# aszepieniec/stark-anatomy

Hardware: AMD Instinct MI355X
Metric: ntt_field_elements_per_sec (higher is better)
Workload: dtype u128; 1 GPU; ntt_fwd_inv_2^20_1gpu; log2n=20, parallelism=single, passes_per_transform=2

## Files before the change

### stark-anatomy_amd/csrc/core.h

```cpp
#pragma once
#include <hip/hip_runtime.h>
#include <dlfcn.h>
#include <cstdio>
#include <cstdlib>
#include <cstring>
#include <algorithm>
#include <atomic>
#include <chrono>
#include <cerrno>
#include <thread>
#include <sys/random.h>
#include <deque>
#include <functional>
#include <future>
#include <map>
#include <mutex>
#include <string>
#include <tuple>
#include <vector>

#pragma GCC visibility push(default)
#include "../../include/starkcore.h"
#pragma GCC visibility pop
#include "ntt_plan.h"

namespace sc { struct FoldIn; }
using namespace sc;

struct sc_vec {
    Fe* d;
    uint64_t n;
    bool owned = true;
};
struct sc_later {
    int slot;
    uint64_t seq;
    hipStream_t st;
};
struct sc_merkle {
    uint64_t* d_levels;
    uint64_t N;
    int logN;
    int slot = -1;
    uint64_t seq = 0;
    hipStream_t st = nullptr;
    bool have_root = false;
    bool lazy = false;
    uint8_t root[64] = {};
};

struct sc_merkle_forest {
    uint64_t* d_levels;
    uint64_t N, count;
    int logN;
    uint64_t* h_roots = nullptr;
    Fe* d_cm = nullptr;
    hipEvent_t done = nullptr;
    hipStream_t st = nullptr;
    bool have_roots = false;
};

namespace sci {

struct DevBuf {
    void* p = nullptr;
    size_t bytes = 0;
};

struct PlanKey {
    int logn;
    uint64_t lo, hi;
    bool operator<(const PlanKey& o) const { return std::tie(logn, lo, hi) < std::tie(o.logn, o.lo, o.hi); }
};
struct PlanTables {
    Fe* mt = nullptr;
    int mt_log = 0;
    Fe* tl = nullptr;
    Fe* th = nullptr;
    Fe* th_ninv = nullptr;
    struct Direct { int logA, logR; bool scaled; Fe* d; };
    std::vector<Direct> direct;
    uint64_t last_use = 0;
};
struct OuterKey {
    uint64_t lo, hi, order, len, batch, col_base;
    int ninv;
    bool operator<(const OuterKey& o) const { return std::tie(lo, hi, order, len, batch, col_base, ninv) < std::tie(o.lo, o.hi, o.order, o.len, o.batch, o.col_base, o.ninv); }
};
struct OuterTable {
    Fe* d = nullptr;
    uint64_t last_use = 0;
};
struct PowKey {
    uint64_t lo, hi, hi_count;
    bool operator<(const PowKey& o) const { return std::tie(lo, hi, hi_count) < std::tie(o.lo, o.hi, o.hi_count); }
};
struct PowTables {
    Fe* lo = nullptr;
    Fe* hi = nullptr;
    uint64_t last_use = 0;
};

struct Ctx {
    bool init = false;
    int device = -1;
    hipStream_t stream = nullptr;
    std::string err;
    NttTuning tuning;
    std::map<PlanKey, PlanTables> plans;
    std::map<PowKey, PowTables> pows;
    std::map<OuterKey, OuterTable> outers;
    uint64_t tick = 0;
    bool foreign_streams = false;
    int small_divisor_direct = 1;
    int div_cols_launch_log = 26;
    int tree_cols_launch_log = 26;
    int eval_chunk_log = 8;
    int eval_points_across_min = 32;
    int eval_across_min_products_log = 26;
    int rescue_tree_split_max_nodes = -1;
    int div_cols_chunk = 0;
    std::vector<hipStream_t> seen_streams;
    DevBuf scratch[8];
    std::map<hipStream_t, DevBuf> ntt_work;
    std::map<hipStream_t, DevBuf> ntt_flags;
    int fast_fixups = 1;
    int num_cus = 256;
    int xcd_remap = 1;
    int fixed_shapes = 1;
    int prio_balance = -1;
    int wave_local = 1;
    unsigned long long* trace = nullptr;
    int forest_four_lane_wgs = 256;
    int merkle_big_nlev = 2;
    int fri_tail = -1;
    int fri_tail_stall = -1;
    size_t verify_stage_bytes = 64ull << 20;
    uint8_t* root_slots = nullptr;
    uint8_t* later_words = nullptr;
    uint64_t root_seq = 0;
    std::vector<int> free_root_slots;
};
constexpr int ROOT_SLOTS = 256;
constexpr size_t ROOT_SLOT_BYTES = 128;
constexpr size_t LATER_WORD_BYTES = 128;
constexpr long SPIN_POLLS = 40000000;

struct PendingFree {
    void* p;
    size_t bytes;
    std::vector<hipEvent_t> evs;
};
#define HIPCHK(expr)                                                                                          \
    do {                                                                                                      \
        hipError_t _e = (expr);                                                                               \
        if (_e != hipSuccess) return fail(SC_ERR_HIP, std::string(#expr) + ": " + hipGetErrorString(_e));     \
    } while (0)

#define SCCHK(expr)              \
    do {                         \
        int _rc = (expr);        \
        if (_rc != SC_OK) return _rc; \
    } while (0)

struct NttOpts {
    uint64_t in_limit = ~0ull;
    const PowTables* coset = nullptr;
    uint32_t cols = 1;
    uint64_t col_stride_in = 0;
};
constexpr uint64_t COLS_ELEMS_PER_LAUNCH = 1ull << 26;
constexpr uint64_t SMALL_DIVISOR = 8;

constexpr uint64_t FUSE_MAX_W = 1ull << 17;

enum BuildMode { BUILD_SYNC = 0, BUILD_ASYNC = 1, BUILD_NOROOT = 2 };

extern Ctx g;
extern std::mutex g_mu;
extern hipStream_t g_comm_stream_for_free;
extern std::future<void> g_rand_worker;
extern size_t g_rand_prefetched;
extern std::multimap<size_t, void*> g_pool;
extern size_t g_pool_bytes, g_pool_cap;
extern std::deque<PendingFree> g_pending;
extern std::vector<hipEvent_t> g_event_pool;

void reap_pending(bool block);
hipError_t pool_alloc(void** p, size_t bytes);
void pool_free(void* p, size_t bytes);
void pool_clear();
hipEvent_t event_get();
int fail(int code, const std::string& msg);
int ensure_init();
int grow_buffer(DevBuf& b, size_t bytes, void** out);
inline int scratch(int slot, size_t bytes, void** out) { return grow_buffer(g.scratch[slot], bytes, out); }
int check_root(Fe root, uint64_t n);
int build_pow_table(Fe** out, uint64_t count, Fe base_m, uint64_t step, Fe scale_m, hipStream_t st);
void free_plans();
int evict_outer_tables();
int get_plan(Fe root, int logn, bool need_ninv, hipStream_t st, PlanTables** out);
inline NttTables tables_of(const PlanTables& t) {
    NttTables tb;
    tb.mt = t.mt; tb.mt_log = t.mt_log; tb.tl = t.tl; tb.th = t.th;
    return tb;
}
int get_pow(Fe base, uint64_t count, hipStream_t st, PowTables** out);
int plan_batched_direct(NttPlanDesc& d, BatchKind kind, int loglen, int logbatch, PlanTables* pt, const Fe* in, Fe* work, Fe* out, BatchExtras ex, hipStream_t st, bool* ok);
int run_plan(NttPlanDesc& d, hipStream_t st);
int ntt_device(const Fe* d_in, Fe* d_out, int logn, Fe root, bool inverse_scale, const NttOpts& o, hipStream_t st);
Fe root_inverse(Fe root, uint64_t n);
int ntt_any(const Fe* d_in, Fe* d_out, uint64_t n, Fe root, bool inverse, const NttOpts& o, hipStream_t st);
int upload(void* d, const void* h, size_t bytes, hipStream_t st);
int download(void* h, const void* d, size_t bytes, hipStream_t st);
int pointwise_div_device(const Fe* a, const Fe* b, Fe* out, uint64_t n, hipStream_t st);
int pointwise_div_enqueue(const Fe* a, const Fe* b, Fe* out, uint64_t n, hipStream_t st, uint32_t* flag);
int gather_device(const Fe* v, const uint64_t* d_idx, uint64_t k, Fe* d_out, hipStream_t st);
int read_small_polled(const void* d_src, size_t bytes, hipStream_t st, void* host_out);
bool upload_small(void* d_dst, const void* host, size_t bytes, hipStream_t st);

int merkle_climb(uint64_t* levels, uint64_t N, int lvl, hipStream_t st, volatile uint64_t* host = nullptr, uint64_t seq = 0, bool* published = nullptr);
int merkle_finish(uint64_t* levels, uint64_t width, hipStream_t st);
int root_slot_get();
int merkle_build_device(const Fe* d_elems, uint64_t N, uint8_t root_out[64], sc_merkle** tree, hipStream_t st, BuildMode mode = BUILD_SYNC, const FoldIn* fold = nullptr);
int merkle_root_wait(sc_merkle* t, bool from_free = false);
void root_poll_unlocked(std::unique_lock<std::mutex>& lk, const sc_merkle* t);
int fold_prepare(const Fe* d_in, uint64_t N, Fe alpha, Fe offset, Fe omega, Fe* d_out, hipStream_t st, FoldIn* f);
int fold_device(const Fe* d_in, uint64_t N, Fe alpha, Fe offset, Fe omega, Fe* d_out, hipStream_t st);
int fold_and_build(const Fe* d_in, uint64_t N, Fe alpha, Fe offset, Fe omega, Fe* d_out, sc_merkle** tree, hipStream_t st);
int fold_constants(uint64_t N, Fe offset, Fe omega, hipStream_t st, PowTables** pw_out, Fe* i2o_m_out);
int host_pool_get(size_t bytes, void** out);
int host_pool_put(void* p);
bool host_pool_holds(const void* p, size_t bytes);
int verify_stage_buffer(size_t bytes, uint8_t** out);

Fe canonical_root(int logn);
Fe ninv_scaled(int logn, int j);
int ntt_cols(const Fe* in, Fe* out, int loglen, int logbatch, bool inverse, hipStream_t st);

constexpr size_t SEEN_STREAMS = 8;
inline hipStream_t pick_stream(void* s) {
    if (s && (hipStream_t)s != g.stream) {
        g.foreign_streams = true;
        hipStream_t st = (hipStream_t)s;
        if (g.seen_streams.size() <= SEEN_STREAMS && std::find(g.seen_streams.begin(), g.seen_streams.end(), st) == g.seen_streams.end())
            g.seen_streams.push_back(st);
    }
    return s ? (hipStream_t)s : g.stream;
}
inline void release_after_streams(void* p, size_t bytes) {
    if (!p) return;
    if (g.seen_streams.size() > SEEN_STREAMS) {
        (void)hipDeviceSynchronize();
        g.seen_streams.clear();
        pool_free(p, bytes);
        return;
    }
    PendingFree f{p, bytes, {}};
    auto mark = [&](hipStream_t st) -> bool {
        if (hipStreamQuery(st) == hipSuccess) return true;
        (void)hipGetLastError();
        hipEvent_t e = event_get();
        if (!e) { (void)hipStreamSynchronize(st); (void)hipGetLastError(); return true; }
        if (hipEventRecord(e, st) != hipSuccess) { (void)hipGetLastError(); g_event_pool.push_back(e); return false; }
        f.evs.push_back(e);
        return true;
    };
    if (g.stream) (void)mark(g.stream);
    if (g_comm_stream_for_free) (void)mark(g_comm_stream_for_free);
    for (size_t i = 0; i < g.seen_streams.size();) {
        if (mark(g.seen_streams[i])) ++i;
        else g.seen_streams.erase(g.seen_streams.begin() + i);
    }
    if (f.evs.empty()) { pool_free(p, bytes); return; }
    g_pending.push_back(std::move(f));
    reap_pending(false);
}
inline Fe fe_from(const uint64_t v[2]) { return Fe{v[0], v[1]}; }
inline bool is_pow2(uint64_t n) { return n && !(n & (n - 1)); }
// ... 29 lines not shown
```

### stark-anatomy_amd/csrc/core.hip

```cpp
#include "core.h"


template <int LOGE> struct PassThreads { static constexpr int value = LOGE >= 4 ? 256 : (LOGE == 3 ? 512 : 1024); };

template <int LOGE>
__global__ void __launch_bounds__(PassThreads<LOGE>::value) ntt_pass_kernel(const PassParams P, uint32_t ntiles, int xcd_remap) {
    extern __shared__ __attribute__((aligned(16))) unsigned char smem_raw[];
    Fe* lds = reinterpret_cast<Fe*>(smem_raw);
    uint32_t wg = blockIdx.x, colbits = 0;
    if (P.col_enable) { colbits = (wg >> P.col_tiles_log) << P.col_tiles_log; wg -= colbits; }
    uint32_t tile = wg;
    if (xcd_remap) tile = (wg & 7u) * (ntiles >> 3) + (wg >> 3);
    tile |= colbits;
    Fe* tw = lds + (1u << (P.logR + P.logC));
    tile_twiddles_to_lds(P, P.logR, threadIdx.x, blockDim.x, tw);
    __syncthreads();
    const int nrounds = (P.logR + LOGE - 1) / LOGE;
    int sh = P.logR;
    for (int r = 0; r < nrounds; ++r) {
        const int s = (r == 0) ? (P.logR - LOGE * (nrounds - 1)) : LOGE;
        sh -= s;
        ntt_round_dispatch<LOGE>(P, s, sh, r == 0, tile, threadIdx.x, lds, tw);
        if (r + 1 < nrounds) __syncthreads();
    }
}

constexpr int TRACE_STAMPS = 16;
template <int LOGE, int GLR, int GLC, bool TRACE, bool ALT = false>
__global__ void __launch_bounds__(1 << (GLR + GLC - LOGE)) ntt_pass_kernel_fixed(const PassParams P, uint32_t ntiles, int xcd_remap, int wave_local) {
    extern __shared__ __attribute__((aligned(16))) unsigned char smem_raw[];
    Fe* lds = reinterpret_cast<Fe*>(smem_raw);
    unsigned long long* trow = nullptr;
    if constexpr (TRACE) {
        if (P.trace) {
            trow = P.trace + ((size_t)blockIdx.x * (blockDim.x >> 6) + (threadIdx.x >> 6)) * TRACE_STAMPS;
            if ((threadIdx.x & 63u) == 0) { trow[0] = __builtin_amdgcn_s_memtime(); trow[15] = __builtin_amdgcn_s_memrealtime(); }
        }
    }
    uint32_t wg = blockIdx.x, colbits = 0;
    if (P.col_enable) { colbits = (wg >> P.col_tiles_log) << P.col_tiles_log; wg -= colbits; }
    uint32_t tile = wg;
    if (xcd_remap) tile = (wg & 7u) * (ntiles >> 3) + (wg >> 3);
    tile |= colbits;
    Fe* tw = lds + (1u << (GLR + GLC));
    auto stamp = [&](int i) {
        if constexpr (TRACE) {
            if (trow) {
                if (i == 2) __builtin_amdgcn_s_waitcnt(0);
                if ((threadIdx.x & 63u) == 0 && i < 13) trow[i] = __builtin_amdgcn_s_memtime();
            }
        }
    };
    auto sync = [] { __syncthreads(); };
    auto wsync = [] { __builtin_amdgcn_fence(__ATOMIC_RELEASE, "wavefront"); __builtin_amdgcn_wave_barrier(); __builtin_amdgcn_fence(__ATOMIC_ACQUIRE, "wavefront"); };
    FixedRounds<LOGE, GLR, GLC, 0, ALT>::run(P, tile, threadIdx.x, lds, tw, sync, wsync, stamp, wave_local != 0);
    if constexpr (TRACE) {
        if (trow && (threadIdx.x & 63u) == 0) { __builtin_amdgcn_s_waitcnt(0); trow[14] = __builtin_amdgcn_s_memtime(); trow[13] = __builtin_amdgcn_s_memrealtime(); }
    }
}

template <int GLR, int GLC>
__device__ __forceinline__ uint32_t fixed8_tile(const PassParams& P, uint32_t index, uint32_t ntiles, int xcd_remap) {
    uint32_t wg = index, colbits = 0;
    if (P.col_enable) { colbits = (wg >> P.col_tiles_log) << P.col_tiles_log; wg -= colbits; }
    uint32_t tile = wg;
    if (xcd_remap) tile = (wg & 7u) * (ntiles >> 3) + (wg >> 3);
    return tile | colbits;
}
template <int GLR, int GLC>
__global__ void __launch_bounds__(1 << (GLR + GLC - 3)) __attribute__((amdgpu_waves_per_eu(4)))
ntt_pass_kernel_fixed8(const PassParams P, uint32_t ntiles, int xcd_remap, int wave_local, uint32_t* flags) {
    extern __shared__ __attribute__((aligned(16))) unsigned char smem_raw[];
    Fe* lds = reinterpret_cast<Fe*>(smem_raw);
    const uint32_t tile = fixed8_tile<GLR, GLC>(P, blockIdx.x, ntiles, xcd_remap);
    Fe* tw = lds + (1u << (GLR + GLC));
    auto stamp = [](int) {};
    auto sync = [] { __syncthreads(); };
    auto wsync = [] { __builtin_amdgcn_fence(__ATOMIC_RELEASE, "wavefront"); __builtin_amdgcn_wave_barrier(); __builtin_amdgcn_fence(__ATOMIC_ACQUIRE, "wavefront"); };
    rare_t rare = 0;
    FixedRounds<3, GLR, GLC, 0, false, true>::run(P, tile, threadIdx.x, lds, tw, sync, wsync, stamp, wave_local != 0, rare);
    if (rare_any(rare)) Round<3, 3, GLR, GLC>::store_word_at(flags + blockIdx.x, 0u, 1u);
}

template <int GLR, int GLC>
__global__ void __launch_bounds__(1 << (GLR + GLC - 3)) __attribute__((amdgpu_waves_per_eu(4)))
ntt_pass_redo8_kernel(const PassParams P, uint32_t ntiles, int xcd_remap, int wave_local, uint32_t* flags, int all) {
    extern __shared__ __attribute__((aligned(16))) unsigned char smem_raw[];
    if (!all && flags[blockIdx.x] == 0) return;
    Fe* lds = reinterpret_cast<Fe*>(smem_raw);
    Fe* tw = lds + (1u << (GLR + GLC));
    auto stamp = [](int) {};
    auto sync = [] { __syncthreads(); };
    auto wsync = [] { __builtin_amdgcn_fence(__ATOMIC_RELEASE, "wavefront"); __builtin_amdgcn_wave_barrier(); __builtin_amdgcn_fence(__ATOMIC_ACQUIRE, "wavefront"); };
    FixedRounds<3, GLR, GLC, 0, false>::run(P, fixed8_tile<GLR, GLC>(P, blockIdx.x, ntiles, xcd_remap), threadIdx.x, lds, tw, sync, wsync, stamp, wave_local != 0);
    if (!all) __syncthreads();
    if (threadIdx.x == 0) flags[blockIdx.x] = 0;
}

__global__ void __launch_bounds__(256) pow_table_kernel(Fe* out, uint64_t count, Fe base_m, uint64_t step, Fe scale_m) {
    uint64_t i = (uint64_t)blockIdx.x * blockDim.x + threadIdx.x;
    if (i < count) out[i] = pow_table_entry(base_m, i, step, scale_m);
}

__global__ void __launch_bounds__(256) twiddle_table_kernel(Fe* out, int logB, uint64_t count, uint64_t scale_exp, const Fe* __restrict__ tl, const Fe* __restrict__ th) {
    uint64_t i = (uint64_t)blockIdx.x * blockDim.x + threadIdx.x;
    if (i >= count) return;
    uint64_t k = i >> logB, b = i & ((1ull << logB) - 1);
    out[i] = pow2level(tl, th, b * k * scale_exp);
}

__global__ void __launch_bounds__(256) pointwise_mul_kernel(const Fe* __restrict__ a, const Fe* __restrict__ b, Fe* __restrict__ out, uint64_t n) {
    uint64_t i = (uint64_t)blockIdx.x * blockDim.x + threadIdx.x;
    if (i < n) out[i] = fe_mul(a[i], b[i]);
}

template <int K>
__global__ void __launch_bounds__(256) pointwise_div_kernel(const Fe* __restrict__ a, const Fe* __restrict__ b, Fe* __restrict__ out, uint64_t n, uint32_t* flag) {
    const uint64_t nthreads = (uint64_t)gridDim.x * blockDim.x;
    const uint64_t t = (uint64_t)blockIdx.x * blockDim.x + threadIdx.x;
    Fe bm[K], pre[K];
    Fe acc = fe_mont_one();
    bool zero = false;
#pragma unroll
    for (int k = 0; k < K; ++k) {
        uint64_t i = t + (uint64_t)k * nthreads;
        Fe v = (i < n) ? b[i] : fe_one();
        zero |= fe_is_zero(v);
        bm[k] = to_mont(v);
        pre[k] = acc;
        acc = mont_mul(acc, bm[k]);
    }
    if (zero) atomicOr(flag, 1u);
    Fe inv = mont_inv(acc);
#pragma unroll
    for (int k = K - 1; k >= 0; --k) {
        uint64_t i = t + (uint64_t)k * nthreads;
        Fe ik = mont_mul(inv, pre[k]);
        inv = mont_mul(inv, bm[k]);
        if (i < n) out[i] = mont_mul(a[i], ik);
    }
}

__global__ void __launch_bounds__(256) short_poly_coset_kernel(const Fe* __restrict__ b, uint32_t nb, Fe off_m, const Fe* __restrict__ tl, const Fe* __restrict__ th, Fe* __restrict__ out, uint64_t order) {
    const uint64_t i = (uint64_t)blockIdx.x * blockDim.x + threadIdx.x;
    if (i >= order) return;
    const Fe x_m = mont_mul(off_m, pow2level(tl, th, i));
    Fe acc = b[nb - 1];
    for (uint32_t k = nb - 1; k-- > 0;) acc = fe_add(mont_mul(acc, x_m), b[k]);
    out[i] = acc;
}

__global__ void __launch_bounds__(256) scale_pow_kernel(const Fe* __restrict__ in, Fe* __restrict__ out, uint64_t n, const Fe* __restrict__ lo, const Fe* __restrict__ hi) {
    uint64_t i = (uint64_t)blockIdx.x * blockDim.x + threadIdx.x;
    if (i < n) out[i] = mont_mul(in[i], pow2level(lo, hi, i));
}

__global__ void __launch_bounds__(256) scale_slab_kernel(const Fe* __restrict__ in, Fe* __restrict__ out, uint64_t rows, int logcols, uint64_t row_len, uint64_t col_base,
                                                         const Fe* __restrict__ lo, const Fe* __restrict__ hi) {
    uint64_t t = (uint64_t)blockIdx.x * blockDim.x + threadIdx.x;
    if (t >= (rows << logcols)) return;
    uint64_t r = t >> logcols, c = t & ((1ull << logcols) - 1);
    out[t] = mont_mul(in[t], pow2level(lo, hi, r * row_len + col_base + c));
}

__global__ void __launch_bounds__(256) axpy_shift_kernel(Fe* __restrict__ acc, const Fe* __restrict__ src, uint64_t n_src, uint64_t shift, Fe w_m) {
    uint64_t j = (uint64_t)blockIdx.x * blockDim.x + threadIdx.x;
    if (j >= n_src) return;
    acc[shift + j] = fe_add(acc[shift + j], mont_mul(src[j], w_m));
}

constexpr int DEGREE_PER_THREAD = 4;
constexpr unsigned DEGREE_MAX_BLOCKS = 2048;
constexpr int DEGREE_SLOTS = 8;
__global__ void __launch_bounds__(256) vec_degree_kernel(const Fe* __restrict__ v, uint64_t n, long long* out) {
    const uint64_t step = (uint64_t)gridDim.x * (256 * DEGREE_PER_THREAD);
    long long best = -1;
    for (uint64_t base = (uint64_t)blockIdx.x * (256 * DEGREE_PER_THREAD) + threadIdx.x; base - threadIdx.x < n; base += step) {
        Fe x[DEGREE_PER_THREAD];
#pragma unroll
        for (int k = 0; k < DEGREE_PER_THREAD; ++k) {
            const uint64_t i = base + 256u * k;
            x[k] = i < n ? v[i] : Fe{0, 0};
        }
#pragma unroll
        for (int k = 0; k < DEGREE_PER_THREAD; ++k) {
            const unsigned long long lanes = __ballot(!fe_is_zero(x[k]));
            if (lanes) best = (long long)(base - (threadIdx.x & 63u) + 256u * k + (63 - __clzll((long long)lanes)));
        }
    }
    __shared__ long long wave_best[4];
    if ((threadIdx.x & 63u) == 0) wave_best[threadIdx.x >> 6] = best;
    __syncthreads();
    if (threadIdx.x == 0) {
        long long m = wave_best[0];
#pragma unroll
        for (int w = 1; w < 4; ++w) m = wave_best[w] > m ? wave_best[w] : m;
        if (m >= 0) atomicMax(out + (blockIdx.x & (DEGREE_SLOTS - 1)), m);
    }
}
__global__ void __launch_bounds__(256) vec_degree_cols_kernel(const Fe* __restrict__ v, uint64_t n, uint64_t ld, uint32_t per_col, long long* out) {
    const uint64_t col = blockIdx.x / per_col;
    const uint32_t part = blockIdx.x - (uint32_t)col * per_col;
    const Fe* __restrict__ w = v + col * ld;
    const uint64_t step = (uint64_t)per_col * (256 * DEGREE_PER_THREAD);
    long long best = -1;
    for (uint64_t base = (uint64_t)part * (256 * DEGREE_PER_THREAD) + threadIdx.x; base - threadIdx.x < n; base += step) {
        Fe x[DEGREE_PER_THREAD];
#pragma unroll
        for (int k = 0; k < DEGREE_PER_THREAD; ++k) {
            const uint64_t i = base + 256u * k;
            x[k] = i < n ? w[i] : Fe{0, 0};
        }
#pragma unroll
        for (int k = 0; k < DEGREE_PER_THREAD; ++k) {
            const unsigned long long lanes = __ballot(!fe_is_zero(x[k]));
            if (lanes) best = (long long)(base - (threadIdx.x & 63u) + 256u * k + (63 - __clzll((long long)lanes)));
        }
    }
    __shared__ long long wave_best[4];
    if ((threadIdx.x & 63u) == 0) wave_best[threadIdx.x >> 6] = best;
    __syncthreads();
    if (threadIdx.x == 0) {
        long long m = wave_best[0];
#pragma unroll
        for (int k = 1; k < 4; ++k) m = wave_best[k] > m ? wave_best[k] : m;
        if (m >= 0) atomicMax(out + col, m);
    }
}
static int degree_read(void* fl, hipStream_t st, long long* deg) {
    long long slots[DEGREE_SLOTS];
    SCCHK(read_small_polled(fl, sizeof slots, st, slots));
    long long m = -1;
    for (int i = 0; i < DEGREE_SLOTS; ++i) m = slots[i] > m ? slots[i] : m;
    *deg = m;
    return SC_OK;
}
static inline unsigned degree_blocks(uint64_t n) {
    const uint64_t b = (n + 256 * DEGREE_PER_THREAD - 1) / (256 * DEGREE_PER_THREAD);
    return (unsigned)(b < DEGREE_MAX_BLOCKS ? (b ? b : 1) : DEGREE_MAX_BLOCKS);
}

__global__ void __launch_bounds__(256) mpoly_eval_kernel(const Fe* __restrict__ vals_m, uint32_t nvars, uint64_t n, const uint8_t* __restrict__ exps,
                                                        const Fe* __restrict__ coef_m, uint32_t nterms, Fe* __restrict__ out, const uint64_t* __restrict__ where) {
    uint64_t i = (uint64_t)blockIdx.x * blockDim.x + threadIdx.x;
    if (i >= n) return;
    Fe acc{0, 0};
    for (uint32_t t = 0; t < nterms; ++t) {
        Fe p = coef_m[t];
        const uint8_t* e = exps + (size_t)t * nvars;
// ... 227 lines not shown
    HIPCHK(hipMalloc((void**)out, count * sizeof(Fe)));
    unsigned blocks = (unsigned)((count + 255) / 256);
    hipLaunchKernelGGL(pow_table_kernel, dim3(blocks), dim3(256), 0, st, *out, count, base_m, step, scale_m);
    HIPCHK(hipGetLastError());
    return SC_OK;
}

void free_plan_tables(PlanTables& t) {
    hipFree(t.mt); hipFree(t.tl); hipFree(t.th);
    if (t.th_ninv) hipFree(t.th_ninv);
    for (const PlanTables::Direct& e : t.direct) hipFree(e.d);
}

void free_plans() {
    for (auto& kv : g.plans) free_plan_tables(kv.second);
    g.plans.clear();
    for (auto& kv : g.pows) { hipFree(kv.second.lo); hipFree(kv.second.hi); }
    g.pows.clear();
    for (auto& kv : g.outers) hipFree(kv.second.d);
    g.outers.clear();
}

constexpr uint64_t PIN_WINDOW = 64;
constexpr size_t PLAN_CAP = 256, POW_CAP = 64;

template <class Map, class FreeFn>
int evict_tables(Map& m, size_t cap, FreeFn free_entry) {
    if (m.size() < cap) return SC_OK;
    std::vector<std::pair<uint64_t, typename Map::iterator>> old;
    for (auto it = m.begin(); it != m.end(); ++it)
        if (it->second.last_use + PIN_WINDOW < g.tick) old.emplace_back(it->second.last_use, it);
    if (old.empty()) return SC_OK;
    std::sort(old.begin(), old.end(), [](const auto& a, const auto& b) { return a.first < b.first; });
    size_t drop = cap / 4 ? cap / 4 : 1;
    if (drop > old.size()) drop = old.size();
    HIPCHK(hipDeviceSynchronize());
    for (size_t i = 0; i < drop; ++i) { free_entry(old[i].second->second); m.erase(old[i].second); }
    return SC_OK;
}

int get_plan(Fe root, int logn, bool need_ninv, hipStream_t st, PlanTables** out) {
    PlanKey key{logn, root.lo, root.hi};
    auto it = g.plans.find(key);
    bool built = false;
    ++g.tick;
    if (it == g.plans.end()) {
        SCCHK(evict_tables(g.plans, PLAN_CAP, free_plan_tables));
        const uint64_t n = 1ull << logn;
        Fe rm = to_mont(root);
        const TableSizes sz = table_sizes(logn);
        PlanTables t;
        t.mt_log = sz.mt_log;
        SCCHK(build_pow_table(&t.mt, sz.mt, rm, n >> sz.mt_log, fe_mont_one(), st));
        SCCHK(build_pow_table(&t.tl, sz.tl, rm, 1, fe_mont_one(), st));
        SCCHK(build_pow_table(&t.th, sz.th, rm, 4096, fe_mont_one(), st));
        it = g.plans.emplace(key, t).first;
        built = true;
    }
    if (need_ninv && !it->second.th_ninv) {
        const uint64_t n = 1ull << logn;
        Fe ninv_m = mont_inv(to_mont(Fe{n, 0}));
        SCCHK(build_pow_table(&it->second.th_ninv, table_sizes(logn).th, to_mont(root), 4096, ninv_m, st));
        built = true;
    }
    if (built) HIPCHK(hipStreamSynchronize(st));
    it->second.last_use = g.tick;
    *out = &it->second;
    return SC_OK;
}

int get_pow(Fe base, uint64_t count, hipStream_t st, PowTables** out) {
    uint64_t hi_count = (count >> 12) + 1;
    uint64_t hc = 1; while (hc < hi_count) hc <<= 1;
    PowKey key{base.lo, base.hi, hc};
    auto it = g.pows.find(key);
    ++g.tick;
    if (it == g.pows.end()) {
        SCCHK(evict_tables(g.pows, POW_CAP, [](PowTables& t) { hipFree(t.lo); hipFree(t.hi); }));
        Fe bm = to_mont(base);
        PowTables t;
        SCCHK(build_pow_table(&t.lo, 4096, bm, 1, fe_mont_one(), st));
        SCCHK(build_pow_table(&t.hi, hc, bm, 4096, fe_mont_one(), st));
        HIPCHK(hipStreamSynchronize(st));
        it = g.pows.emplace(key, t).first;
    }
    it->second.last_use = g.tick;
    *out = &it->second;
    return SC_OK;
}

int direct_twiddles(PlanTables* pt, const NttPlanDesc& d, int i, bool scaled, hipStream_t st, const Fe** out) {
    const DirectTable t = direct_table(d, i, scaled);
    *out = nullptr;
    if (t.logR + t.logB > g.tuning.direct_tw_max_log) return SC_OK;
    for (const PlanTables::Direct& e : pt->direct)
        if (e.logA == t.logA && e.logR == t.logR && e.scaled == t.scaled) { *out = e.d; return SC_OK; }
    const uint64_t count = 1ull << (t.logR + t.logB);
    Fe* p;
    HIPCHK(hipMalloc((void**)&p, count * sizeof(Fe)));
    pt->direct.push_back({t.logA, t.logR, t.scaled, p});
    hipLaunchKernelGGL(twiddle_table_kernel, dim3((unsigned)((count + 255) / 256)), dim3(256), 0, st, p, t.logB, count, 1ull << t.logA,
                       pt->tl, t.scaled ? pt->th_ninv : pt->th);
    HIPCHK(hipGetLastError());
    HIPCHK(hipStreamSynchronize(st));
    *out = p;
    return SC_OK;
}

int plan_batched_direct(NttPlanDesc& d, BatchKind kind, int loglen, int logbatch, PlanTables* pt, const Fe* in, Fe* work, Fe* out, BatchExtras ex, hipStream_t st, bool* ok) {
    const NttTables tb = tables_of(*pt);
    *ok = plan_batched(d, kind, loglen, logbatch, tb, in, work, out, g.tuning, ex);
    if (!*ok || d.npasses != 2) return SC_OK;
    SCCHK(direct_twiddles(pt, d, 0, false, st, &ex.inner_twd));
    if (ex.inner_twd) *ok = plan_batched(d, kind, loglen, logbatch, tb, in, work, out, g.tuning, ex);
    return SC_OK;
}

int pass_flags(hipStream_t st, uint32_t nwg, uint32_t** out) {
    DevBuf& b = g.ntt_flags[st];
    const void* before = b.p;
    const size_t had = b.bytes;
    void* p;
    SCCHK(grow_buffer(b, (size_t)nwg * sizeof(uint32_t), &p));
    if (p != before || b.bytes != had) HIPCHK(hipMemsetAsync(p, 0, b.bytes, st));
    *out = (uint32_t*)p;
    return SC_OK;
}

template <int LOGE>
int launch_pass(const NttPassDesc& pd, hipStream_t st) {
    int remap = (g.xcd_remap && pd.ntiles >= 16 && (pd.ntiles & 7u) == 0) ? 1 : 0;
    const PassKernel k = pass_kernel(pd, g.fixed_shapes != 0);
    if constexpr (LOGE == 2) {
        if (k.kind == PK_FIXED4) {
            const int lr = pd.p.logR, lc = pd.p.logC;
#define SC_LAUNCH_FIXED(LR, LC, TR, ALT) \
    hipLaunchKernelGGL((ntt_pass_kernel_fixed<2, LR, LC, TR, ALT>), dim3(pd.ntiles * pd.cols), dim3(pd.threads), pd.lds_bytes, st, pd.p, pd.ntiles, remap, g.wave_local)
#define SC_FIXED(LR, LC)                                                          \
            if (lr == LR && lc == LC) {                                           \
                if (k.trace) SC_LAUNCH_FIXED(LR, LC, true, false);                \
                else if (k.alt) SC_LAUNCH_FIXED(LR, LC, false, true);             \
                else SC_LAUNCH_FIXED(LR, LC, false, false);                       \
                return SC_OK;                                                     \
            }
            SC_FIXED4_SHAPES(SC_FIXED)
#undef SC_FIXED
        }
    }
    if constexpr (LOGE == 3) {
        if (k.kind == PK_FIXED8) {
            const int lr = pd.p.logR, lc = pd.p.logC;
            const uint32_t nwg = pd.ntiles * pd.cols;
            const bool fast = g.fast_fixups != 0 && fast_pass_ok(pd.p) && !pass_in_place(pd);
            const int all = (!fast || g.fast_fixups == 2) ? 1 : 0;
            uint32_t* flags;
            SCCHK(pass_flags(st, nwg, &flags));
#define SC_FIXED8(LR, LC)                                                                                                                                   \
            if (lr == LR && lc == LC) {                                                                                                                     \
                if (fast) hipLaunchKernelGGL((ntt_pass_kernel_fixed8<LR, LC>), dim3(nwg), dim3(pd.threads), pd.lds_bytes, st, pd.p, pd.ntiles, remap, g.wave_local, flags); \
                hipLaunchKernelGGL((ntt_pass_redo8_kernel<LR, LC>), dim3(nwg), dim3(pd.threads), pd.lds_bytes, st, pd.p, pd.ntiles, remap, g.wave_local, flags, all); \
                return SC_OK;                                                                                                                               \
            }
            SC_FIXED8_SHAPES(SC_FIXED8)
#undef SC_FIXED8
        }
    }
    hipLaunchKernelGGL(ntt_pass_kernel<LOGE>, dim3(pd.ntiles * pd.cols), dim3(pd.threads), pd.lds_bytes, st, pd.p, pd.ntiles, remap);
    return SC_OK;
}

int run_plan(NttPlanDesc& d, hipStream_t st) {
    size_t trace_off = 0;
    for (int i = 0; i < d.npasses; ++i) {
        d.pass[i].p.prio_balance = pass_prio_balance(d.pass[i], g.prio_balance, g.num_cus);
        d.pass[i].p.trace = g.trace ? g.trace + trace_off : nullptr;
        trace_off += (size_t)d.pass[i].ntiles * d.pass[i].cols * (d.pass[i].threads >> 6) * TRACE_STAMPS;
        switch (d.pass[i].loge) {
            case 1: SCCHK(launch_pass<1>(d.pass[i], st)); break;
            case 2: SCCHK(launch_pass<2>(d.pass[i], st)); break;
            case 3: SCCHK(launch_pass<3>(d.pass[i], st)); break;
            case 4: SCCHK(launch_pass<4>(d.pass[i], st)); break;
            default: return fail(SC_ERR_UNSUPPORTED, "bad loge");
        }
        HIPCHK(hipGetLastError());
    }
    return SC_OK;
}

int ntt_device(const Fe* d_in, Fe* d_out, int logn, Fe root, bool inverse_scale, const NttOpts& o, hipStream_t st) {
    PlanTables* pt;
    SCCHK(get_plan(root, logn, inverse_scale, st, &pt));
    const uint64_t n = 1ull << logn;
    const int m = plan_num_passes(logn, g.tuning);
    NttTables tb = tables_of(*pt);
    tb.th_scaled = (inverse_scale && m > 1) ? pt->th_ninv : nullptr;
    NttIo io;
    io.in = d_in; io.out = d_out; io.in_limit = o.in_limit; io.cols = o.cols; io.col_stride_in = o.col_stride_in;
    if (m > 1) { void* w; SCCHK(grow_buffer(g.ntt_work[st], n * o.cols * sizeof(Fe), &w)); io.work = (Fe*)w; }
    if (o.coset) { io.ol = o.coset->lo; io.oh = o.coset->hi; }
    if (inverse_scale && m == 1) { io.scale_last = true; io.scale = mont_inv(to_mont(Fe{n, 0})); }
    NttPlanDesc d;
    if (!plan_ntt(d, logn, tb, io, g.tuning)) return fail(SC_ERR_UNSUPPORTED, "unsupported transform length");
    if (d.npasses > 1) {
        bool any = false;
        for (int i = 0; i + 1 < d.npasses; ++i) {
            SCCHK(direct_twiddles(pt, d, i, inverse_scale, st, &tb.twd[i]));
            any |= tb.twd[i] != nullptr;
        }
        if (any && !plan_ntt(d, logn, tb, io, g.tuning)) return fail(SC_ERR_UNSUPPORTED, "unsupported transform length");
    }
    return run_plan(d, st);
}

Fe root_inverse(Fe root, uint64_t n) {
    return from_mont(mont_pow(to_mont(root), n - 1));
}

int ntt_any(const Fe* d_in, Fe* d_out, uint64_t n, Fe root, bool inverse, const NttOpts& o, hipStream_t st) {
    if (n <= 1) {
        if (n == 1 && d_in != d_out) HIPCHK(hipMemcpyAsync(d_out, d_in, sizeof(Fe), hipMemcpyDeviceToDevice, st));
        return SC_OK;
    }
    if (!is_pow2(n)) return fail(SC_ERR_NOT_POW2, "cannot compute ntt of non-power-of-two sequence");
    SCCHK(check_root(root, n));
    return ntt_device(d_in, d_out, ilog2(n), inverse ? root_inverse(root, n) : root, inverse, o, st);
}

int upload(void* d, const void* h, size_t bytes, hipStream_t st) {
    if (bytes) HIPCHK(hipMemcpyAsync(d, h, bytes, hipMemcpyHostToDevice, st));
    return SC_OK;
}
int download(void* h, const void* d, size_t bytes, hipStream_t st) {
    if (bytes) HIPCHK(hipMemcpyAsync(h, d, bytes, hipMemcpyDeviceToHost, st));
    HIPCHK(hipStreamSynchronize(st));
    return SC_OK;
}

int pointwise_div_enqueue(const Fe* a, const Fe* b, Fe* out, uint64_t n, hipStream_t st, uint32_t* flag) {
    HIPCHK(hipMemsetAsync(flag, 0, 8, st));
    static const int K = [] { const char* e = getenv("STARKCORE_DIV_K"); return e && atoi(e) == 8 ? 8 : 16; }();
    const uint64_t threads = (n + K - 1) / K;
    const unsigned blocks = (unsigned)((threads + 255) / 256);
    if (K == 8) hipLaunchKernelGGL(pointwise_div_kernel<8>, dim3(blocks), dim3(256), 0, st, a, b, out, n, flag);
    else hipLaunchKernelGGL(pointwise_div_kernel<16>, dim3(blocks), dim3(256), 0, st, a, b, out, n, flag);
    HIPCHK(hipGetLastError());
    return SC_OK;
}
int pointwise_div_device(const Fe* a, const Fe* b, Fe* out, uint64_t n, hipStream_t st) {
    void* fl;
    SCCHK(scratch(4, 256, &fl));
    SCCHK(pointwise_div_enqueue(a, b, out, n, st, (uint32_t*)fl));
    uint64_t hflag = 0;
    SCCHK(read_small_polled(fl, 8, st, &hflag));
    if ((uint32_t)hflag) return fail(SC_ERR_DIV_ZERO, "divide by zero");
    return SC_OK;
}

__global__ void __launch_bounds__(64) words_publish_kernel(const uint64_t* __restrict__ src, uint32_t nwords, volatile uint64_t* host, uint64_t seq) {
    if (threadIdx.x < nwords) host[threadIdx.x] = src[threadIdx.x];
    __threadfence_system();
    if (threadIdx.x == 0) host[8] = seq;
}
int read_small_polled(const void* d_src, size_t bytes, hipStream_t st, void* host_out) {
    const int slot = (bytes <= 64 && ((uintptr_t)d_src & 7) == 0) ? root_slot_get() : -1;
    if (slot < 0) {
        HIPCHK(hipMemcpyAsync(host_out, d_src, bytes, hipMemcpyDeviceToHost, st));
        HIPCHK(hipStreamSynchronize(st));
        return SC_OK;
    }
    const uint64_t seq = ++g.root_seq;
    volatile uint64_t* host = (volatile uint64_t*)(g.root_slots + ROOT_SLOT_BYTES * slot);
    hipLaunchKernelGGL(words_publish_kernel, dim3(1), dim3(64), 0, st, (const uint64_t*)d_src, (uint32_t)((bytes + 7) / 8), host, seq);
    hipError_t e = hipGetLastError();
    bool landed = false;
    if (e == hipSuccess) {
        for (long spin = 0; spin < SPIN_POLLS; ++spin) {
            if (__atomic_load_n(host + 8, __ATOMIC_ACQUIRE) == seq) { landed = true; break; }
            if ((spin & 4095) == 4095) {
                e = hipStreamQuery(st);
                if (e != hipErrorNotReady) break;
                (void)hipGetLastError();
                e = hipSuccess;
            }
        }
        if (!landed) {
            (void)hipGetLastError();
            e = hipStreamSynchronize(st);
            landed = e == hipSuccess && __atomic_load_n(host + 8, __ATOMIC_ACQUIRE) == seq;
            if (e == hipSuccess && !landed) e = hipErrorUnknown;
        }
    }
    if (landed) memcpy(host_out, (const void*)host, bytes);
    else (void)hipStreamSynchronize(st);
    g.free_root_slots.push_back(slot);
    if (!landed) return fail(SC_ERR_HIP, hipGetErrorString(e));
    return SC_OK;
}

static int later_words(int slot, uint32_t** zero_flag, long long** degree_slots) {
    if (!g.later_words) HIPCHK(hipMalloc((void**)&g.later_words, LATER_WORD_BYTES * ROOT_SLOTS));
    uint8_t* w = g.later_words + LATER_WORD_BYTES * slot;
    *degree_slots = (long long*)w;
    *zero_flag = (uint32_t*)(w + DEGREE_SLOTS * sizeof(long long));
    return SC_OK;
}
__global__ void __launch_bounds__(64) divide_flags_publish_kernel(const uint32_t* __restrict__ zero_flag, const long long* __restrict__ degree_slots,
                                                                 volatile uint64_t* host, uint64_t seq) {
    if (threadIdx.x == 0) {
        long long m = -1;
        if (degree_slots) for (int i = 0; i < DEGREE_SLOTS; ++i) m = degree_slots[i] > m ? degree_slots[i] : m;
        host[0] = zero_flag ? (uint64_t)*zero_flag : 0ull;
        host[1] = (uint64_t)m;
        __threadfence_system();
        host[8] = seq;
    }
}
static int divide_flags_later(int slot, const uint32_t* zero_flag, const long long* degree_slots, hipStream_t st, sc_later** out) {
    const uint64_t seq = ++g.root_seq;
    volatile uint64_t* host = (volatile uint64_t*)(g.root_slots + ROOT_SLOT_BYTES * slot);
    hipLaunchKernelGGL(divide_flags_publish_kernel, dim3(1), dim3(64), 0, st, zero_flag, degree_slots, host, seq);
    HIPCHK(hipGetLastError());
    *out = new sc_later{slot, seq, st};
    return SC_OK;
}
static int later_abandon(int slot, hipStream_t st, int rc) {
    (void)hipStreamSynchronize(st);
    g.free_root_slots.push_back(slot);
    return rc;
}
int later_wait(sc_later* h, uint64_t words[8]) {
    volatile uint64_t* host = (volatile uint64_t*)(g.root_slots + ROOT_SLOT_BYTES * h->slot);
    bool landed = false;
    hipError_t e = hipSuccess;
    for (long spin = 0; spin < SPIN_POLLS; ++spin) {
        if (__atomic_load_n(host + 8, __ATOMIC_ACQUIRE) == h->seq) { landed = true; break; }
        if ((spin & 4095) == 4095) {
            e = hipStreamQuery(h->st);
            if (e != hipErrorNotReady) break;
            (void)hipGetLastError();
            e = hipSuccess;
        }
    }
    if (!landed) {
        (void)hipGetLastError();
        e = hipStreamSynchronize(h->st);
        landed = e == hipSuccess && __atomic_load_n(host + 8, __ATOMIC_ACQUIRE) == h->seq;
        if (e == hipSuccess && !landed) e = hipErrorUnknown;
    }
    if (landed) memcpy(words, (const void*)host, 64);
    g.free_root_slots.push_back(h->slot);
    delete h;
    if (!landed) return fail(SC_ERR_HIP, hipGetErrorString(e));
    return SC_OK;
}

int gather_device(const Fe* v, const uint64_t* d_idx, uint64_t k, Fe* d_out, hipStream_t st) {
    hipLaunchKernelGGL(gather_kernel, dim3((unsigned)((k + 255) / 256)), dim3(256), 0, st, v, d_idx, k, d_out);
    HIPCHK(hipGetLastError());
    return SC_OK;
}

int evict_outer_tables() { return evict_tables(g.outers, (size_t)16, [](OuterTable& t) { hipFree(t.d); }); }

}


extern "C" {

int sc_device_count(void) {
    int n = 0;
    if (hipGetDeviceCount(&n) != hipSuccess) return 0;
    return n;
}

int sc_init(int device) {
    std::lock_guard<std::mutex> lk(g_mu);
    if (g.init && (device < 0 || device == g.device)) return SC_OK;
    if (g.init) return fail(SC_ERR_BAD_ARG, "already initialised on another device");
    if (device >= 0) { char buf[16]; snprintf(buf, sizeof buf, "%d", device); setenv("STARKCORE_DEVICE", buf, 1); }
    return ensure_init();
}

int sc_shutdown(void) {
    std::lock_guard<std::mutex> lk(g_mu);
    if (g_rand_worker.valid()) { g_rand_worker.get(); g_rand_prefetched = 0; }
    if (!g.init) return SC_OK;
    hipDeviceSynchronize();
    reap_pending(true);
    for (hipEvent_t e : g_event_pool) (void)hipEventDestroy(e);
    g_event_pool.clear();
    free_plans();
    pool_clear();
    for (auto& b : g.scratch) { if (b.p) hipFree(b.p); b = DevBuf{}; }
    for (auto& kv : g.ntt_work) if (kv.second.p) hipFree(kv.second.p);
    g.ntt_work.clear();
    for (auto& kv : g.ntt_flags) if (kv.second.p) hipFree(kv.second.p);
    g.ntt_flags.clear();
    if (g.later_words) hipFree(g.later_words);
    g.later_words = nullptr;
    if (g.stream) hipStreamDestroy(g.stream);
    g.stream = nullptr;
    g.seen_streams.clear();
    g.foreign_streams = false;
    g.init = false;
    return SC_OK;
}

const char* sc_last_error(void) { return g.err.c_str(); }

int sc_synchronize(void) {
    std::lock_guard<std::mutex> lk(g_mu);
    SCCHK(ensure_init());
    HIPCHK(hipStreamSynchronize(g.stream));
    return SC_OK;
}

int sc_stream(void** stream_out) {
    std::lock_guard<std::mutex> lk(g_mu);
    SCCHK(ensure_init());
    if (!stream_out) return fail(SC_ERR_BAD_ARG, "null argument");
    *stream_out = (void*)g.stream;
    return SC_OK;
}

int sc_stream_join(void* other) {
    std::lock_guard<std::mutex> lk(g_mu);
    SCCHK(ensure_init());
    hipStream_t o = (hipStream_t)other;
    if (o == g.stream) return SC_OK;
    (void)pick_stream(other);
    hipEvent_t a = event_get(), b = event_get();
    if (!a || !b) { if (a) g_event_pool.push_back(a); if (b) g_event_pool.push_back(b); HIPCHK(hipStreamSynchronize(o)); HIPCHK(hipStreamSynchronize(g.stream)); return SC_OK; }
    hipError_t e = hipEventRecord(a, o);
    if (e == hipSuccess) e = hipStreamWaitEvent(g.stream, a, 0);
    if (e == hipSuccess) e = hipEventRecord(b, g.stream);
    if (e == hipSuccess) e = hipStreamWaitEvent(o, b, 0);
    g_event_pool.push_back(a);
    g_event_pool.push_back(b);
    if (e != hipSuccess) return fail(SC_ERR_HIP, hipGetErrorString(e));
    return SC_OK;
}

int sc_set_tuning(const char* key, int value) {
    std::lock_guard<std::mutex> lk(g_mu);
    std::string k(key ? key : "");
    if (k == "max_tile_log") g.tuning.max_tile_log = value;
    else if (k == "loge") g.tuning.loge = value;
    else if (k == "max_col_log") g.tuning.max_col_log = value;
    else if (k == "min_tiles_log") g.tuning.min_tiles_log = value;
    else if (k == "single_pass_max_log") g.tuning.single_pass_max_log = value;
    else if (k == "max_digit_log") g.tuning.max_digit_log = value;
    else if (k == "direct_tw_max_log") g.tuning.direct_tw_max_log = value;
    else if (k == "xcd_remap") g.xcd_remap = value;
    else if (k == "fixed_shapes") g.fixed_shapes = value;
    else if (k == "wave_local") g.wave_local = value;
    else if (k == "fast_fixups") g.fast_fixups = value < 0 ? 0 : (value > 2 ? 2 : value);
    else if (k == "prio_balance") g.prio_balance = value;
    else if (k == "loge_cols") g.tuning.loge_cols = value;
    else if (k == "tw_on_load") g.tuning.tw_on_load = value;
    else if (k == "prune") g.tuning.prune = value;
    else if (k == "merkle_big_nlev") g.merkle_big_nlev = value < 0 ? 0 : (value > 8 ? 8 : value);
    else if (k == "forest_four_lane_wgs") g.forest_four_lane_wgs = value < 0 ? 0 : value;
    else if (k == "fri_tail") g.fri_tail = value ? 1 : 0;
    else if (k == "small_divisor_direct") g.small_divisor_direct = value ? 1 : 0;
    else if (k == "div_cols_chunk") g.div_cols_chunk = value < 0 ? 0 : (value > 65535 ? 65535 : value);
    else if (k == "div_cols_launch_log") g.div_cols_launch_log = value < 1 ? 1 : (value > 26 ? 26 : value);
    else if (k == "tree_cols_launch_log") g.tree_cols_launch_log = value < 1 ? 1 : (value > 26 ? 26 : value);
    else if (k == "eval_chunk_log") g.eval_chunk_log = value < 8 ? 8 : (value > 24 ? 24 : value);
    else if (k == "eval_points_across_min") g.eval_points_across_min = value < 1 ? 1 : value;
    else if (k == "eval_across_min_products_log") g.eval_across_min_products_log = value < 0 ? 0 : (value > 64 ? 64 : value);
    else if (k == "rescue_tree_split_max_nodes") g.rescue_tree_split_max_nodes = value < -1 ? -1 : value;
    else if (k == "verify_stage_kb") g.verify_stage_bytes = (size_t)(value < 16 ? 16 : value) << 10;
    else if (k == "fri_tail_stall") g.fri_tail_stall = value;
    else if (k == "pool_cap_mb") g_pool_cap = (size_t)(value < 0 ? 0 : value) << 20;
    else if (k == "pool_trim") {
        if (g.init) { (void)hipDeviceSynchronize(); reap_pending(true); pool_clear(); }
    }
    else return fail(SC_ERR_BAD_ARG, "unknown tuning key " + k);
    return SC_OK;
}

int sc_ntt_num_passes(uint64_t n) {
    std::lock_guard<std::mutex> lk(g_mu);
    if (n < 2 || !is_pow2(n)) return 0;
    return plan_num_passes(ilog2(n), g.tuning);
}

int sc_debug_trace(void* d_buf) {
    std::lock_guard<std::mutex> lk(g_mu);
    g.trace = (unsigned long long*)d_buf;
    return SC_OK;
}

int sc_vec_alloc(uint64_t n, sc_vec_t** out) {
    std::lock_guard<std::mutex> lk(g_mu);
    SCCHK(ensure_init());
    sc_vec* v = new sc_vec{nullptr, n};
    hipError_t e = pool_alloc((void**)&v->d, (n ? n : 1) * sizeof(Fe));
    if (e != hipSuccess) { delete v; return fail(SC_ERR_HIP, hipGetErrorString(e)); }
    *out = v;
    return SC_OK;
}
int sc_vec_free(sc_vec_t* v) {
    std::lock_guard<std::mutex> lk(g_mu);
    if (!v) return SC_OK;
    if (v->owned) release_after_streams(v->d, (v->n ? v->n : 1) * sizeof(Fe));
    delete v;
    return SC_OK;
}
int sc_vec_wrap(void* d_elems, uint64_t n, sc_vec_t** out) {
    if (!d_elems || !out) return fail(SC_ERR_BAD_ARG, "null argument");
    sc_vec* v = new sc_vec{(Fe*)d_elems, n};
    v->owned = false;
    *out = v;
    return SC_OK;
}
uint64_t sc_vec_len(const sc_vec_t* v) { return v ? v->n : 0; }
void* sc_vec_ptr(sc_vec_t* v) { return v ? v->d : nullptr; }
int sc_vec_zero(sc_vec_t* v) {
    std::lock_guard<std::mutex> lk(g_mu);
    if (!v) return fail(SC_ERR_BAD_ARG, "null vector");
    SCCHK(ensure_init());
    if (v->n) HIPCHK(hipMemsetAsync(v->d, 0, v->n * sizeof(Fe), g.stream));
    return SC_OK;
}
}
namespace sci {
struct SmallPayload { uint64_t w[256]; };
__global__ void __launch_bounds__(256) small_upload_kernel(uint64_t* __restrict__ dst, const SmallPayload p, uint32_t nwords) {
    if (threadIdx.x < nwords) dst[threadIdx.x] = p.w[threadIdx.x];
}
bool upload_small(void* d_dst, const void* host, size_t bytes, hipStream_t st) {
    if (bytes > 4 * sizeof(SmallPayload)) return false;
    const uint8_t* src = (const uint8_t*)host;
    uint64_t* dst = (uint64_t*)d_dst;
    for (size_t left = bytes; left;) {
        const size_t take = left < sizeof(SmallPayload) ? left : sizeof(SmallPayload);
        SmallPayload p;
        p.w[(take - 1) / 8] = 0;
        memcpy(p.w, src, take);
        hipLaunchKernelGGL(small_upload_kernel, dim3(1), dim3(256), 0, st, dst, p, (uint32_t)((take + 7) / 8));
        src += take; dst += (take + 7) / 8; left -= take;
    }
    return hipGetLastError() == hipSuccess;
}
}
extern "C" {
int sc_vec_upload(sc_vec_t* v, uint64_t offset, const void* host, uint64_t count) {
    std::lock_guard<std::mutex> lk(g_mu);
    SCCHK(ensure_init());
    if (!v || offset + count > v->n) return fail(SC_ERR_BAD_ARG, "upload out of range");
    if (count && upload_small(v->d + offset, host, count * sizeof(Fe), g.stream)) return SC_OK;
    SCCHK(upload(v->d + offset, host, count * sizeof(Fe), g.stream));
    HIPCHK(hipStreamSynchronize(g.stream));
    return SC_OK;
}
int sc_vec_download(const sc_vec_t* v, uint64_t offset, void* host, uint64_t count) {
    std::lock_guard<std::mutex> lk(g_mu);
    SCCHK(ensure_init());
    if (!v || offset + count > v->n) return fail(SC_ERR_BAD_ARG, "download out of range");
    return download(host, v->d + offset, count * sizeof(Fe), g.stream);
}
int sc_sample_bytes_dev(const void* bytes, uint64_t count, uint32_t width, void* d_out, void* stream) {
    std::lock_guard<std::mutex> lk(g_mu);
    SCCHK(ensure_init());
    if (!count) return SC_OK;
    if (!bytes || !d_out || width == 0 || width > 32) return fail(SC_ERR_BAD_ARG, "byte strings of 1..32 bytes expected");
    hipStream_t st = pick_stream(stream);
    void* buf;
    SCCHK(scratch(6, count * width + 256, &buf));
    SCCHK(upload(buf, bytes, count * width, st));
    hipLaunchKernelGGL(sample_bytes_kernel, dim3((unsigned)((count + 255) / 256)), dim3(256), 0, st, (const uint8_t*)buf, count, width, (Fe*)d_out);
    HIPCHK(hipGetLastError());
    HIPCHK(hipStreamSynchronize(st));
    return SC_OK;
}
namespace {
uint8_t* g_rand_host = nullptr;
size_t g_rand_host_bytes = 0;
hipEvent_t g_rand_copied = nullptr;
std::atomic<int> g_rand_failed{0};

void rand_fill(size_t bytes) {
    unsigned hw = std::thread::hardware_concurrency();
    size_t nthreads = bytes / (256u << 10);
    if (nthreads > 32) nthreads = 32;
    if (hw && nthreads > hw) nthreads = hw;
    static const long cap = [] { const char* e = getenv("STARKCORE_RAND_THREADS"); return e ? atol(e) : 0L; }();
    if (cap > 0 && nthreads > (size_t)cap) nthreads = (size_t)cap;
    if (nthreads < 1) nthreads = 1;
    auto fill = [](size_t a, size_t b) {
        while (a < b) {
            size_t want = b - a < (1u << 20) ? b - a : (1u << 20);
            ssize_t r = getrandom(g_rand_host + a, want, 0);
            if (r < 0) { if (errno == EINTR) continue; g_rand_failed = 1; return; }
            a += (size_t)r;
        }
    };
    if (nthreads == 1) { fill(0, bytes); return; }
    std::vector<std::thread> pool;
    const size_t per = (bytes + nthreads - 1) / nthreads;
    for (size_t i = 0; i < nthreads; ++i) {
        const size_t a = i * per, b = a + per < bytes ? a + per : bytes;
        if (a < b) pool.emplace_back(fill, a, b);
    }
    for (auto& t : pool) t.join();
}
uint8_t* g_rand_dev = nullptr;
size_t g_rand_dev_bytes = 0;
// ... 568 lines not shown
```

Measured before the change: 49.45 billion field-elements/s.

## Replace per-tile redo launch with persistent grid-strided repair kernel

The fast pass kernel flags tiles needing a rare fixup. Previously a redo kernel was launched over every workgroup, and most of them just read a flag and exited. Now a small persistent grid (about two workgroups per CU) scans the flags with a wave ballot and reprocesses only the flagged tiles through a noinline device function. This is meant to remove the cost of dispatching many empty workgroups, at the cost of serialising any real repairs within a group and using extra registers for the noinline call.

After: 49.81 billion field-elements/s (median of 6 runs). About the same (+0.7%).

```diff
diff --git a/stark-anatomy_amd/csrc/core.h b/stark-anatomy_amd/csrc/core.h
--- a/stark-anatomy_amd/csrc/core.h
+++ b/stark-anatomy_amd/csrc/core.h
@@ -125,6 +125,7 @@
     std::map<hipStream_t, DevBuf> ntt_work;
     std::map<hipStream_t, DevBuf> ntt_flags;
     int fast_fixups = 1;
+    int redo_groups = 0;
     int num_cus = 256;
     int xcd_remap = 1;
     int fixed_shapes = 1;
diff --git a/stark-anatomy_amd/csrc/core.hip b/stark-anatomy_amd/csrc/core.hip
--- a/stark-anatomy_amd/csrc/core.hip
+++ b/stark-anatomy_amd/csrc/core.hip
@@ -84,17 +84,51 @@
 
 template <int GLR, int GLC>
 __global__ void __launch_bounds__(1 << (GLR + GLC - 3)) __attribute__((amdgpu_waves_per_eu(4)))
-ntt_pass_redo8_kernel(const PassParams P, uint32_t ntiles, int xcd_remap, int wave_local, uint32_t* flags, int all) {
+ntt_pass_redo8_kernel(const PassParams P, uint32_t ntiles, int xcd_remap, int wave_local, uint32_t* flags) {
     extern __shared__ __attribute__((aligned(16))) unsigned char smem_raw[];
-    if (!all && flags[blockIdx.x] == 0) return;
     Fe* lds = reinterpret_cast<Fe*>(smem_raw);
     Fe* tw = lds + (1u << (GLR + GLC));
     auto stamp = [](int) {};
     auto sync = [] { __syncthreads(); };
     auto wsync = [] { __builtin_amdgcn_fence(__ATOMIC_RELEASE, "wavefront"); __builtin_amdgcn_wave_barrier(); __builtin_amdgcn_fence(__ATOMIC_ACQUIRE, "wavefront"); };
     FixedRounds<3, GLR, GLC, 0, false>::run(P, fixed8_tile<GLR, GLC>(P, blockIdx.x, ntiles, xcd_remap), threadIdx.x, lds, tw, sync, wsync, stamp, wave_local != 0);
-    if (!all) __syncthreads();
     if (threadIdx.x == 0) flags[blockIdx.x] = 0;
+}
+
+template <int GLR, int GLC>
+__device__ __attribute__((noinline)) void repair8_tile(uint32_t kernarg_lo_v, uint32_t kernarg_hi_v, uint32_t tile_v, uint32_t wave_local_v) {
+    extern __shared__ __attribute__((aligned(16))) unsigned char smem_raw[];
+    typedef const __attribute__((address_space(4))) PassParams* KernargParams;
+    const uint32_t kernarg_lo = __builtin_amdgcn_readfirstlane(kernarg_lo_v), kernarg_hi = __builtin_amdgcn_readfirstlane(kernarg_hi_v);
+    const uint64_t kernarg = (uint64_t)kernarg_lo | ((uint64_t)kernarg_hi << 32);
+    const PassParams& P = *(const PassParams*)(KernargParams)kernarg;
+    const uint32_t tile = __builtin_amdgcn_readfirstlane(tile_v);
+    const bool wave_local = __builtin_amdgcn_readfirstlane(wave_local_v) != 0;
+    Fe* lds = reinterpret_cast<Fe*>(smem_raw);
+    Fe* tw = lds + (1u << (GLR + GLC));
+    auto stamp = [](int) {};
+    auto sync = [] { __syncthreads(); };
+    auto wsync = [] { __builtin_amdgcn_fence(__ATOMIC_RELEASE, "wavefront"); __builtin_amdgcn_wave_barrier(); __builtin_amdgcn_fence(__ATOMIC_ACQUIRE, "wavefront"); };
+    FixedRounds<3, GLR, GLC, 0, false>::run(P, tile, threadIdx.x, lds, tw, sync, wsync, stamp, wave_local);
+}
+template <int GLR, int GLC>
+__global__ void __launch_bounds__(1 << (GLR + GLC - 3)) __attribute__((amdgpu_waves_per_eu(4)))
+ntt_pass_repair8_kernel(const PassParams P, uint32_t ntiles, int xcd_remap, int wave_local, uint32_t* flags, uint32_t nwg, uint32_t groups) {
+    const uint32_t b = blockIdx.x;
+    const uint32_t count = (nwg - b + groups - 1) / groups;
+    const uint32_t lane = threadIdx.x & 63u;
+    const uint64_t kernarg = (uint64_t)__builtin_amdgcn_kernarg_segment_ptr();
+    for (uint32_t base = 0; base < count; base += 64u) {
+        const uint32_t k = base + lane;
+        uint64_t mask = __ballot(k < count && flags[b + groups * k] != 0);
+        while (mask) {
+            const uint32_t index = b + groups * (base + (uint32_t)__builtin_ctzll(mask));
+            mask &= mask - 1;
+            repair8_tile<GLR, GLC>((uint32_t)kernarg, (uint32_t)(kernarg >> 32), fixed8_tile<GLR, GLC>(P, index, ntiles, xcd_remap), (uint32_t)wave_local);
+            __syncthreads();
+            if (threadIdx.x == 0) flags[index] = 0;
+        }
+    }
 }
 
 __global__ void __launch_bounds__(256) pow_table_kernel(Fe* out, uint64_t count, Fe base_m, uint64_t step, Fe scale_m) {
@@ -628,13 +662,15 @@
             const int lr = pd.p.logR, lc = pd.p.logC;
             const uint32_t nwg = pd.ntiles * pd.cols;
             const bool fast = g.fast_fixups != 0 && fast_pass_ok(pd.p) && !pass_in_place(pd);
-            const int all = (!fast || g.fast_fixups == 2) ? 1 : 0;
+            const bool repair = fast && g.fast_fixups == 1;
+            const uint32_t groups = std::min(nwg, g.redo_groups > 0 ? (uint32_t)g.redo_groups : 2u * (uint32_t)std::max(g.num_cus, 1));
             uint32_t* flags;
             SCCHK(pass_flags(st, nwg, &flags));
 #define SC_FIXED8(LR, LC)                                                                                                                                   \
             if (lr == LR && lc == LC) {                                                                                                                     \
                 if (fast) hipLaunchKernelGGL((ntt_pass_kernel_fixed8<LR, LC>), dim3(nwg), dim3(pd.threads), pd.lds_bytes, st, pd.p, pd.ntiles, remap, g.wave_local, flags); \
-                hipLaunchKernelGGL((ntt_pass_redo8_kernel<LR, LC>), dim3(nwg), dim3(pd.threads), pd.lds_bytes, st, pd.p, pd.ntiles, remap, g.wave_local, flags, all); \
+                if (repair) hipLaunchKernelGGL((ntt_pass_repair8_kernel<LR, LC>), dim3(groups), dim3(pd.threads), pd.lds_bytes, st, pd.p, pd.ntiles, remap, g.wave_local, flags, nwg, groups); \
+                else hipLaunchKernelGGL((ntt_pass_redo8_kernel<LR, LC>), dim3(nwg), dim3(pd.threads), pd.lds_bytes, st, pd.p, pd.ntiles, remap, g.wave_local, flags); \
                 return SC_OK;                                                                                                                               \
             }
             SC_FIXED8_SHAPES(SC_FIXED8)
@@ -931,6 +967,7 @@
     else if (k == "fixed_shapes") g.fixed_shapes = value;
     else if (k == "wave_local") g.wave_local = value;
     else if (k == "fast_fixups") g.fast_fixups = value < 0 ? 0 : (value > 2 ? 2 : value);
+    else if (k == "redo_groups") g.redo_groups = value < 0 ? 0 : value;
     else if (k == "prio_balance") g.prio_balance = value;
     else if (k == "loge_cols") g.tuning.loge_cols = value;
     else if (k == "tw_on_load") g.tuning.tw_on_load = value;
```
